# rpng/open_vins

Hardware: AMD Instinct MI355X
Metric: MSCKF features/sec per EKF update (30-clone state) (higher is better)
Workload: dtype f64; 1 GPU; BASELINE.json configs[2]: 2-camera radtan rig, 30-clone window, 2000 MSCKF features/update, N=248, D=208, online cam extrinsic+intrinsic calib + IMU intrinsics in the state, FEJ; features_total=2000, features_this_rank=2000, clones=30, cameras=2, state_dim=248, measurements_total=100362, parallelism=single GPU

## Files before the change

open_vins_amd/csrc/api_context.inc:

```
using namespace ovg;

static thread_local std::string g_err = "";
static int set_err(int code, const std::string &msg) {
  g_err = msg;
  return code;
}

#define HIPCHK(expr)                                                                                         \
  do {                                                                                                       \
    hipError_t _e = (expr);                                                                                  \
    if (_e != hipSuccess) {                                                                                  \
      return set_err(OVGPU_ERR_HIP, std::string(#expr) + " -> " + hipGetErrorString(_e) + " (" __FILE__ ":" + \
                                        std::to_string(__LINE__) + ")");                                     \
    }                                                                                                        \
  } while (0)

namespace {

struct AllocCount {
  std::atomic<int64_t> n{0}, bytes{0};
  void add(size_t b) { n.fetch_add(1, std::memory_order_relaxed), bytes.fetch_add((int64_t)b, std::memory_order_relaxed); }
  void sub(size_t b) { n.fetch_sub(1, std::memory_order_relaxed), bytes.fetch_sub((int64_t)b, std::memory_order_relaxed); }
};
struct DeviceAlloc {
// ... 354 lines not shown
  int chol_spin_limit = 1 << 22;
  int chol_timeouts = 0;
  int mode_a_factor = 0;
  bool factor_from_gram = false;
  bool last_factor_from_gram = false;
  int last_gram_kernel = 0, last_factor_kernel = 0, last_unwhiten_kernel = 0;
  bool chol_timed_out = false;
  bool prior_pending = false;
  bool prior_overlap = true;
  const double *last_uinv = nullptr;
  const double *prior_uinv = nullptr;
  int layout_fpw = 8;
  bool unwhiten_blocked = true;
  bool pchol_blocked = true;
  bool speculative_prior = true;
  DevBuf<int32_t> gram_dropped;
  DevView<int32_t> rows_used;
  DevBuf<double> sys_rows_ws;
  int row_stride = 48;

  std::vector<EventPair> ev_compress, ev_update, ev_system;
  size_t ev_used = 0;
  bool timed_this_update = false;
  bool timing = true;
  int timing_period = 1;
  uint64_t timing_seq = 0;
};

static Batch batch_of(const ovgpu_ctx *c) {
  if (c->view) return *c->view;
// ... 164 lines not shown
```

open_vins_amd/csrc/api_debug.inc:

```
int ovgpu_debug_option(ovgpu_ctx *c, const char *name, int64_t value, int64_t *old_value) {
  if (!c || !name) return set_err(OVGPU_ERR_INVALID, "null argument");
  const std::string n(name);
  if (n == "chol_follow_spin_limit") {
    if (old_value) *old_value = c->chol_spin_limit;
    if (value >= 0) c->chol_spin_limit = (int)std::min<int64_t>(value, 1 << 30);
  } else if (n == "slam_chunked_fail_chunk") {
    if (old_value) *old_value = c->chunk_fail_inject;
    c->chunk_fail_inject = value >= 0 ? (int)std::min<int64_t>(value, 1 << 20) : -1;
  } else if (n == "slam_chunked_fallbacks") {
    if (old_value) *old_value = c->chunk_fallbacks;
    if (value >= 0) c->chunk_fallbacks = value;
  } else if (n == "delayed_init_fused") {
    if (old_value) *old_value = c->init_fused;
    if (value >= 0) c->init_fused = (int)std::min<int64_t>(value, 2);
  } else if (n == "delayed_init_fused_steps") {
    if (old_value) *old_value = c->init_fused_steps;
    if (value >= 0) c->init_fused_steps = value;
  } else if (n == "delayed_init_rows_steps") {
    if (old_value) *old_value = c->init_rows_steps;
    if (value >= 0) c->init_rows_steps = value;
  } else if (n == "delayed_init_chain_steps") {
    if (old_value) *old_value = c->init_chain_steps;
    if (value >= 0) c->init_chain_steps = value;
  } else if (n == "gram_interleaved") {
    if (old_value) *old_value = c->gram_il ? 1 : 0;
    if (value >= 0) c->gram_il = value != 0;
  } else if (n == "layout_fpw") {
    if (old_value) *old_value = c->layout_fpw;
    if (value >= 1 && value <= 8) c->layout_fpw = (int)value;
  } else if (n == "unwhiten_blocked") {
    if (old_value) *old_value = c->unwhiten_blocked ? 1 : 0;
    if (value >= 0) c->unwhiten_blocked = value != 0;
  } else if (n == "pchol_blocked") {
    if (old_value) *old_value = c->pchol_blocked ? 1 : 0;
    if (value >= 0) c->pchol_blocked = value != 0;
  } else if (n == "speculative_prior") {
    if (old_value) *old_value = c->speculative_prior ? 1 : 0;
    if (value >= 0) c->speculative_prior = value != 0;
  } else if (n == "raw_stack") {
    if (old_value) *old_value = c->raw_enable ? 1 : 0;
    if (value >= 0) c->raw_enable = value != 0, c->raw_one_region = value == 2;
  } else if (n == "anchored_fast") {
    if (old_value) *old_value = c->anchored_fast ? 1 : 0;
    if (value >= 0) c->anchored_fast = value != 0;
  } else if (n == "slam_fused") {
    if (old_value) *old_value = c->slam_fused;
    if (value >= 0) c->slam_fused = (int)std::min<int64_t>(value, 3);
  } else if (n == "slam_fused_batches") {
    if (old_value) *old_value = c->slam_fused_batches;
    if (value >= 0) c->slam_fused_batches = value;
  } else if (n == "gram_blocks_only") {
    if (old_value) *old_value = c->gram_blocks_only ? 1 : 0;
    if (value >= 0) c->gram_blocks_only = value != 0;
// ... 279 lines not shown
```

open_vins_amd/csrc/api_pipeline.inc:

```
static int enqueue_triangulate(ovgpu_ctx *c, const double *seed_pA = nullptr, const int32_t *seed_anchor = nullptr) {
  const Batch b = batch_of(c);
  if (b.F == 0) return OVGPU_OK;
  TriParams p;
  p.seed_pA = seed_pA, p.seed_anchor = seed_anchor, p.anchor_pre = c->anchor_pre.p;
  p.F = b.F, p.C = c->C, p.K = c->K;
  p.meas_offsets = b.meas_offsets, p.meas_cc = b.meas_cc, p.uvn = b.uvn, p.tab_cc = c->tab_cc.p;
  p.p_FinA = b.pA, p.p_FinG = b.pG, p.anchor_meas = c->anchor.p, p.status = b.status;
  p.opt = c->dopt;
  const size_t lds = (size_t)c->K * c->C * 12 * sizeof(double);
  if (lds > (size_t)c->lds_limit) {
    return set_err(OVGPU_ERR_CAPACITY, "k_triangulate: the pose table of K = " + std::to_string(c->K) + " cameras x C = " + std::to_string(c->C) + " clones (96 bytes a pair, " +
                                           std::to_string(lds) + " bytes) exceeds the LDS limit of " + std::to_string(c->lds_limit) + " bytes");
  }
  int wpb = c->tri_waves;
  if (wpb == 0) {
    wpb = 4;
    const int room = c->num_cu - 6;
    for (int w = 4; w <= 8 && room > 0; w *= 2) {
      const int blocks = (b.F + w - 1) / w;
      if (blocks <= room) {
        if (4 * blocks >= 3 * room) wpb = w;
        break;
      }
    }
  }
  hipLaunchKernelGGL(with_max_lds<k_triangulate>(c), dim3((b.F + wpb - 1) / wpb), dim3(64 * wpb), lds, c->stream, p);
  HIPCHK(hipGetLastError());
  return OVGPU_OK;
}

struct FeatLaunch {
  FeatKernel kernel = FK_GENERAL;
  FeatKernel code = FK_GENERAL;
  bool f32 = false;
  bool ch = false;
  bool alt = false;
  int cb = 0;
  size_t lds = 0;
// ... 100 lines not shown

static int enqueue_system(ovgpu_ctx *c, int f_one = -1, int init_rep = 0, bool whiten = false) {
  const Batch b = batch_of(c);
  if (b.F == 0) return OVGPU_OK;
  SysParams p;
  fill_sys_params(c, b, p);
  c->stack_is_f32 = false;
  p.Lw = (whiten && f_one < 0) ? c->Lw.p : nullptr;
  c->last_stack_raw = false;
  if (f_one < 0) c->last_feat_kernel = FK_GENERAL;
  if (f_one < 0) HIPCHK(ctrl_zero(c, CTRL_ROWS, c->rows_used.p, 2 * sizeof(int32_t), c->stream));
  if (f_one >= 0) sys_params_init_mode(c, p, f_one, init_rep);
  const FeatLaunch s = select_feat_kernel(c, p, b.F, f_one);
  if (s.err != OVGPU_OK) return set_err(s.err, s.msg);
  if (s.cb) {
    p.row_stride = 48;
    HIPCHK(ctrl_zero(c, CTRL_COUNTER, c->feat_counter.p, sizeof(int32_t), c->stream));
    p.work_counter = c->feat_counter.p;
    feat::FeatStore st{c->fs_rows.p, c->fs_minfo.p, c->fs_V.p, c->fs_z.p, c->fs_meas_feat.p, c->fs_w.p, c->fs_pos.p};
    if (s.f32) {
      c->stack_ldf = ((c->LD + 31) / 32) * 32;
      HIPCHK(c->Hbig32.reserve((size_t)(std::max<int64_t>(b.rows_total, 1) + 32) * c->stack_ldf));
      HIPCHK(hipMemsetAsync(c->Hbig32.p + (size_t)b.rows_total * c->stack_ldf, 0, sizeof(float) * 32 * c->stack_ldf, c->stream));
      p.Hbig32 = c->Hbig32.p, p.LDF = c->stack_ldf;
      c->stack_is_f32 = true;
    }
    if (p.opt.feat_rep >= OVGPU_REP_ANCHORED_3D) hipLaunchKernelGGL(feat::k_feat_rows_anchored, dim3((b.M + 255) / 256), dim3(256), 0, c->stream, p, st, b.M);
    else hipLaunchKernelGGL(feat::k_feat_rows_sorted, dim3((b.M + 255) / 256), dim3(256), 0, c->stream, p, st, b.M);
    if (c->raw_enable && c->raw_tables_ok && !c->raw_veto && s.kernel != FK_FEATY_BIG && !s.f32 && s.cb == feat::FY_CB) {
      p.raw.on = 1, p.raw.ncls = c->raw_ncls, p.raw.H = c->Hraw.p, p.raw.dst = c->raw_dst.p, p.raw.j0 = c->raw_j0;
// ... 442 lines not shown
      sp = c->stream2;
      c->prior_on_side = true;
    }
    const int64_t elems = (int64_t)D * LA;
    const bool at_source = c->fuse_chol_inputs && chol_pipe_usable(c, D);
    if (!at_source) hipLaunchKernelGGL(k_tf_gather, dim3((unsigned)((elems + 255) / 256)), dim3(256), 0, sp, t);
    p.diag0 = c->gram_rho.p, p.pivot_tol = c->prior_pivot_tol;
    CholSource from;
    if (at_source) from.src = chol::CH_SRC_PRIOR, from.t = &t;
    c->last_uinv = nullptr;
    if ((rc = enqueue_chol_carry(c, p, sp, c->Lw.p, from)) != OVGPU_OK) return rc;
    c->prior_uinv = c->last_uinv;
    p.diag0 = nullptr;
    if (c->prior_on_side) HIPCHK(hipEventRecord(c->ev_join, sp));
    c->prior_pending = true;
  }
  if (part & 2) {
    if (c->prior_on_side) HIPCHK(hipStreamWaitEvent(s, c->ev_join, 0));
    c->prior_pending = false, c->prior_on_side = false;
    p.pred = c->flags.p + 3;
    CholSource from;
    if (t.whitened && c->fuse_chol_inputs && chol_pipe_usable(c, D)) {
      from.src = chol::CH_SRC_WHITENED, from.t = &t;
      p.pred = nullptr, p.pred_not = c->flags.p;
    } else if (t.whitened) {
      hipLaunchKernelGGL(k_tf_abh, dim3((D + 3) / 4), dim3(256), 0, s, t, (const int32_t *)c->flags.p, c->flags.p + 3);
    } else {
      hipLaunchKernelGGL(k_tf_go, dim3(1), dim3(1), 0, s, (const int32_t *)c->flags.p, c->flags.p + 3);
      hipLaunchKernelGGL(k_tf_w, dim3((tm * tm + 3) / 4), dim3(256), 0, s, t);
      hipLaunchKernelGGL(k_tf_t, dim3((tm * tm + 3) / 4), dim3(256), 0, s, t);
// ... 536 lines not shown
```

open_vins_amd/csrc/api_standalone.inc:

```
int ovgpu_measurement_compress(ovgpu_ctx *c, int rows, int cols, const double *H, const double *res, double *H_out, double *res_out, int32_t *rows_out) {
  if (!c) return set_err(OVGPU_ERR_INVALID, "null ctx");
  if (rows <= cols) {
    if (H_out && H && H_out != H) std::memcpy(H_out, H, sizeof(double) * (size_t)rows * cols);
    if (res_out && res && res_out != res) std::memcpy(res_out, res, sizeof(double) * rows);
    if (rows_out) *rows_out = rows;
    return OVGPU_OK;
  }
  DenseJob job(c);
  int rc = dense_compress(c, rows, cols, H, res);
  if (rc != OVGPU_OK) return rc;
  const int LD = cols + 1;
  std::vector<double> tri((size_t)cols * LD);
  HIPCHK(hipMemcpyAsync(tri.data(), c->Rws.p, sizeof(double) * tri.size(), hipMemcpyDeviceToHost, c->stream));
  HIPCHK(upload_sync(c, c->stream));
  for (int i = 0; i < cols; i++) {
    if (H_out) std::memcpy(H_out + (size_t)i * cols, &tri[(size_t)i * LD], sizeof(double) * cols);
    if (res_out) res_out[i] = tri[(size_t)i * LD + cols];
  }
  if (rows_out) *rows_out = cols;
  return check_tree_error(c);
}

int ovgpu_ekf_update(ovgpu_ctx *c, int rows, int cols, const int32_t *col_cov_id, const double *H, const double *res, double sigma2, double *dx,
                     double *P_out) {
// ... 56 lines not shown
  if (!c || !n_doubles) return set_err(OVGPU_ERR_INVALID, "null argument");
  if (!c->have_state || c->poses_only) return set_err(OVGPU_ERR_NO_STATE, "ovgpu_set_state was never called");
  const int NT = (c->LD + 15) / 16;
  if (NT > gram::GR_NT_BLK) return set_err(OVGPU_ERR_CAPACITY, "the Gram route holds at most 383 Jacobian columns");
  *n_doubles = (int64_t)256 * NT * NT + 1;
  return OVGPU_OK;
}

int ovgpu_msckf_local_gram(ovgpu_ctx *c, int32_t *feat_status, double *chi2, double *chi2_thresh, double *p_FinG, void *gram_dev,
                           ovgpu_update_stats *stats) {
  if (!c || !gram_dev) return set_err(OVGPU_ERR_INVALID, "null argument");
  if (stats) std::memset(stats, 0, sizeof(*stats));
  if (!c->have_state || c->poses_only) return set_err(OVGPU_ERR_NO_STATE, "ovgpu_set_state was never called");
  HIPCHK(hipSetDevice(c->device));
  int rc = OVGPU_OK;
  c->prior_pending = false;
  rc = enqueue_pipeline(c, STAGE_LOCAL, false, true, true);
  if (rc != OVGPU_OK) return rc;
  const size_t n = (size_t)256 * ((c->LD + 15) / 16) * ((c->LD + 15) / 16);
  double *dst = static_cast<double *>(gram_dev);
  if (batch_of(c).F > 0) {
    HIPCHK(hipMemcpyAsync(dst, c->gram_G.p, sizeof(double) * n, hipMemcpyDeviceToDevice, c->stream));
    hipLaunchKernelGGL(k_gram_count, dim3(1), dim3(1), 0, c->stream, dst + n, c->rows_used.p);
    HIPCHK(hipGetLastError());
  } else {
    HIPCHK(hipMemsetAsync(dst, 0, sizeof(double) * (n + 1), c->stream));
    c->gram_is_whitened = c->whiten;
  }
  if (feat_status || chi2 || chi2_thresh || p_FinG || stats) {
    rc = read_feature_outputs(c, feat_status, chi2, chi2_thresh, p_FinG, stats);
    if (rc != OVGPU_OK) return rc;
// ... 128 lines not shown
```

open_vins_amd/csrc/api_state.inc:

```

const char *ovgpu_last_error(void) { return g_err.c_str(); }

void ovgpu_default_options(ovgpu_options *o) {
  if (!o) return;
  std::memset(o, 0, sizeof(*o));
  o->chi2_multipler = 5.0, o->sigma_pix = 1.0;
  o->triangulate_1d = 0, o->refine_features = 1, o->max_runs = 5;
  o->init_lamda = 1e-3, o->max_lamda = 1e10, o->min_dx = 1e-6, o->min_dcost = 1e-6, o->lam_mult = 10;
  o->min_dist = 0.10, o->max_dist = 60, o->max_baseline = 40, o->max_cond_number = 10000;
  o->do_fej = 1, o->do_calib_camera_pose = 1, o->do_calib_camera_intrinsics = 1;
  o->feat_rep_msckf = OVGPU_REP_GLOBAL_3D;
}

double ovgpu_chi2_quantile_95(int dof) { return chi2_quantile_95(dof); }
int ovgpu_abi_version(void) { return OVGPU_ABI_VERSION; }

static int init_context(ovgpu_ctx *c, const ovgpu_options *opts, int device) {
  c->device = device;
  c->opts = *opts;
  hipDeviceProp_t prop;
  HIPCHK(hipGetDeviceProperties(&prop, device));
  c->num_cu = prop.multiProcessorCount > 0 ? prop.multiProcessorCount : 256;
  c->lds_limit = (int)std::min<size_t>(prop.sharedMemPerBlock, 160 * 1024);
  HIPCHK(hipStreamCreateWithFlags(&c->stream.h, hipStreamNonBlocking));
// ... 379 lines not shown
  std::vector<double> tab((size_t)12 * K * C);
  for (int i = 0; i < K * C; i++) {
    std::memcpy(&tab[(size_t)12 * i], R_GtoC + (size_t)9 * i, 9 * sizeof(double));
    std::memcpy(&tab[(size_t)12 * i + 9], p_CinG + (size_t)3 * i, 3 * sizeof(double));
  }
  HIPCHK(c->tab_cc.reserve(tab.size()));
  HIPCHK(upload(c->tab_cc.p, tab.data(), sizeof(double) * tab.size(), c->stream));
  HIPCHK(upload_sync(c, c->stream));
  c->C = C, c->K = K, c->N = 0, c->D = 0, c->LD = 1, c->L = 0;
  c->have_state = true, c->poses_only = true, c->have_feats = false, c->tri_readable = false;
  return OVGPU_OK;
}

static bool featy_block_rows(const ovgpu_ctx *c) { return c->plan.msckf == FK_FEATY_BIG || c->featy_big; }
static int featy_block_cols(const ovgpu_ctx *c) { return featy_block_rows(c) ? 32 : feat::FY_CB; }
static int enqueue_batch_layout(ovgpu_ctx *c, bool anchors, int cb) {
  const Batch b = batch_of(c);
  const int F = b.F;
  const bool fast = c->plan.msckf != FK_GENERAL && b.M > 0;
  if (F > 0 && (anchors || fast)) {
    const int m_max = feat::batch_layout_m_pad(std::max(b.m_max, 1));
    const size_t lds_one = feat::batch_layout_lds_ints(m_max) * sizeof(int32_t);
    int fpw_want = 1;
    while (fpw_want < std::min(c->layout_fpw, (int)feat::BL_FPW) && (F + fpw_want - 1) / fpw_want > 250) fpw_want *= 2;
    const int fpw = fast ? std::max(1, std::min<int>(fpw_want, (int)((48 * 1024) / lds_one))) : 1;
    const size_t lds = fast ? (size_t)fpw * lds_one : 0;
    const bool raw_tabs = fast && c->raw_tables_ok;
    RawStack rw;
    for (int k = 0; k <= RAW_NEG; k++) rw.base[k] = c->raw_base[k], rw.ld[k] = c->raw_ld[k], rw.rcol[k] = c->raw_rcol[k];
    hipLaunchKernelGGL(feat::k_batch_layout, dim3((F + fpw - 1) / fpw), dim3(fast ? feat::BL_NTH * fpw : 64), lds, c->stream, F, m_max, c->D, (const int32_t *)b.meas_offsets, (const uint16_t *)b.meas_cc,
                       (const int32_t *)c->clone_col.p, (const int32_t *)c->calib_col.p, (const int32_t *)c->intr_col.p, anchors ? c->anchor_pre.p : (int32_t *)nullptr,
                       fast ? c->fs_meas_feat.p : (int32_t *)nullptr, fast ? c->fs_pos.p : (int32_t *)nullptr, fast ? c->fs_inst.p : (int32_t *)nullptr, c->plan.nt, cb, c->C, c->K,
                       (const uint8_t *)c->cls_of_clone.p, (const int32_t *)c->raw_featbase.p, raw_tabs ? c->raw_dst.p : (int32_t *)nullptr,
                       raw_tabs ? c->raw_runs.p : (int32_t *)nullptr, rw);
    HIPCHK(hipGetLastError());
  }
  c->inst_cb = fast ? cb : 0, c->inst_D = c->D;
  return OVGPU_OK;
}
static int enqueue_instance_lists(ovgpu_ctx *c, int cb) { return enqueue_batch_layout(c, false, cb); }
static int enqueue_batch_tables(ovgpu_ctx *c, bool anchors) { return enqueue_batch_layout(c, anchors, c->plan.msckf != FK_GENERAL ? featy_block_cols(c) : feat::FY_CB); }

static int feature_rows(bool slam_rows, int m, int proj) { return slam_rows ? std::max(2 * m - proj, 0) : (m >= 2 ? 2 * m - 3 : 0); }
static void row_offsets_of(const ovgpu_ctx *c, const Batch &b, bool slam_rows, int64_t *out) {
  const int udof = lm_uniform_dof(c);
  out[0] = 0;
  for (int f = 0; f < b.F; f++) {
    int proj = udof == 1 ? 2 : 0;
    if (udof == 0 && (int)b.h_feat_lm.size() == b.F) proj = 3 - lm_dof(c->h_lm_rep[b.h_feat_lm[f]]);
    out[f + 1] = out[f] + feature_rows(slam_rows, b.h_offsets[f + 1] - b.h_offsets[f], proj);
  }
}
static void track_order(const int32_t *offsets, int F, int m_max, int32_t *order) {
  std::vector<int32_t> start(m_max + 2, 0);
  for (int f = 0; f < F; f++) start[m_max - (offsets[f + 1] - offsets[f]) + 1]++;
  for (int b = 0; b <= m_max; b++) start[b + 1] += start[b];
// ... 150 lines not shown
      r.chunk_begin = (int)((nchunks * j) / w), r.chunk_end = (int)((nchunks * (j + 1)) / w);
      r.part_tile = tiles, r.region = (c->raw_rs.n - 1) | (k == RAW_NEG ? 16 : 0);
      tiles += r.ntc * (r.ntc + 1) / 2;
      tab.push_back(r);
    }
  }
  c->gram_wg_n = (int)tab.size(), c->gram_wg_tiles = tiles;
  HIPCHK(c->gram_wg.reserve(tab.size()));
  HIPCHK(c->up.put(c->gram_wg.p, tab.data(), sizeof(gram::GramRegionWG) * tab.size()));
  c->raw_tables_ok = true;
  return OVGPU_OK;
}

static int begin_feature_batch(ovgpu_ctx *c, int F, int M, const int32_t *offsets) {
  c->have_feats = false, c->tri_readable = false;
  c->raw_tables_ok = false;
  int m_max = 0;
  for (int f = 0; f < F; f++) {
    const int m = offsets[f + 1] - offsets[f];
    if (m < 0) return set_err(OVGPU_ERR_INVALID, "meas_offsets not monotone");
    m_max = std::max(m_max, m);
  }
  c->F = F, c->M = M, c->m_max = m_max;
  c->have_feat_sigma = c->have_feat_mult = false;
  c->h_feat_lm.clear(), c->h_feat_rep.clear();
  c->h_offsets.assign(offsets, offsets + (F > 0 ? F + 1 : 0));
  if (F == 0) c->h_offsets.assign(1, 0);

  const int need = std::max(500, 2 * m_max + 1);
  if ((int)c->h_chi2_table.size() < need) {
// ... 87 lines not shown
```

open_vins_amd/csrc/k_featy.h:

```cpp
#pragma once
#include <type_traits>

#include "k_feat.h"

namespace ovg {
namespace feat {

#ifdef OVG_FEAT_ABLATE
#define FY_SKIP(p) ((p).skip)
#else
#define FY_SKIP(p) 0
#endif
#ifndef FY_SYRK_UNROLL
#define FY_SYRK_UNROLL 2
#endif
constexpr int FY_CB = 64;
constexpr int FY_LS = 66;

struct FeatYLds {
  size_t yb, vl, wpart, misc, raw, total;
};
__host__ __device__ inline FeatYLds featy_lds_layout(int nt_max, int nta_max, int nw, int cb) {
  FeatYLds L;
  size_t o = 0;
// ... 132 lines not shown
        p.raw.H[off + (int64_t)(r & 1) * ld + rcol] = res[r];
      }
      if (lane < 4) {
        const double cr = lane < 3 && lane < n ? res[lane] - (V[3 * lane] * z0 + V[3 * lane + 1] * z1 + V[3 * lane + 2] * z2) : 0.0;
        p.raw.H[p.raw.base[RAW_NEG] + ((int64_t)4 * f + lane) * p.raw.ld[RAW_NEG] + p.raw.rcol[RAW_NEG]] = cr;
      }
    }
    if (lane == 0) tq[(size_t)8 * f + 6] = sumsq / p.opt.sigma_pix_sq;
  }
}

__host__ __device__ inline int batch_layout_m_pad(int m_max) { return (m_max + 15) & ~15; }
__host__ __device__ inline size_t batch_layout_lds_ints(int m_pad) { return (size_t)4 * m_pad + (size_t)((2 * m_pad + 15) >> 4) * 48; }
constexpr int BL_NTH = 128, BL_TR = BL_NTH / 24;
constexpr int BL_FPW = 8;
__global__ void __launch_bounds__(BL_NTH * BL_FPW) k_batch_layout(int F, int m_max, int D, const int32_t *__restrict__ meas_offsets, const uint16_t *__restrict__ meas_cc,
                                                      const int32_t *__restrict__ clone_col, const int32_t *__restrict__ calib_col, const int32_t *__restrict__ intr_col,
                                                      int32_t *__restrict__ anchor_pre, int32_t *__restrict__ meas_feat, int32_t *__restrict__ pos, int32_t *__restrict__ inst,
                                                      int nt_max, int cb, int C, int K, const uint8_t *__restrict__ cls_of_clone, const int32_t *__restrict__ featbase,
                                                      int32_t *__restrict__ raw_dst, int32_t *__restrict__ raw_runs, RawStack rw) {
  extern __shared__ __attribute__((aligned(16))) unsigned char smem_all[];
  const int gth = min((int)blockDim.x, BL_NTH), grp = threadIdx.x / gth;
  const int tid = threadIdx.x - grp * gth, lane = tid & 63, wv = tid >> 6;
  const int f = blockIdx.x * ((int)blockDim.x / gth) + grp;
  const bool active = f < F;
  unsigned char *smem = smem_all + (size_t)grp * batch_layout_lds_ints(m_max) * sizeof(int32_t);
  __shared__ int tab_clone[1024], tab_calib[64], tab_intr[64];
  __shared__ uint8_t tab_cls[1024];
  __shared__ int grp_nt[BL_FPW];
  __shared__ __attribute__((aligned(16))) int cls_cnt[BL_FPW][RAW_MAXCLS];
  if (pos) {
    if (raw_runs && tid < RAW_MAXCLS) cls_cnt[grp][tid] = 0;
    for (int i = threadIdx.x; i < C; i += blockDim.x) tab_clone[i] = clone_col[i];
    if (raw_dst)
      for (int i = threadIdx.x; i < C; i += blockDim.x) tab_cls[i] = cls_of_clone[i];
    if (threadIdx.x < K) tab_calib[threadIdx.x] = calib_col[threadIdx.x], tab_intr[threadIdx.x] = intr_col[threadIdx.x];
  }
  const int m0 = active ? meas_offsets[f] : 0, m = active ? meas_offsets[f + 1] - m0 : 0;
  if (pos && tid == 0) grp_nt[grp] = (2 * m + 15) >> 4;
  if (anchor_pre && active && wv == (gth >> 6) - 1) {
    long long best = -1;
    int best_end = -1, carry_start = 0;
    for (int base = 0; base < m; base += 64) {
      const int i = base + lane;
      const bool valid = i < m;
      const int cam = valid ? (int)(meas_cc[m0 + i] >> 10) : -1;
      const int prev = (valid && i > 0) ? (int)(meas_cc[m0 + i - 1] >> 10) : -2;
      const int next = (valid && i + 1 < m) ? (int)(meas_cc[m0 + i + 1] >> 10) : -3;
      const unsigned long long starts = __ballot(valid && cam != prev);
      if (valid && cam != next) {
        const unsigned long long below = starts & (lane == 63 ? ~0ull : ((2ull << lane) - 1ull));
        const int start = below ? base + 63 - __clzll((long long)below) : carry_start;
        const long long key = ((long long)(i - start + 1) << 32) | (long long)(0x7fffffff - start);
        if (key > best) best = key, best_end = i;
      }
      if (starts) carry_start = base + 63 - __clzll((long long)starts);
    }
#pragma unroll
    for (int off = 32; off >= 1; off >>= 1) {
      const long long ob = __shfl_xor(best, off);
      const int oe = __shfl_xor(best_end, off);
      if (ob > best) best = ob, best_end = oe;
    }
    if (lane == 0) anchor_pre[f] = best_end >= 0 ? m0 + best_end : -1;
  }
  if (!pos) return;
  typedef int i32x4 __attribute__((ext_vector_type(4)));
  int *keys = reinterpret_cast<int *>(smem);
  int *cols3 = keys + m_max;
  int *cand = cols3 + 3 * m_max;
  const int NT = (2 * m + 15) >> 4;
  int *kept = cand + 24 * ((2 * m_max + 15) >> 4);
  __syncthreads();
  for (int i = tid; i < ((m + 15) & ~15); i += BL_NTH) {
    int key = 0x7fffffff;
    if (i < m) {
      const int code = meas_cc[m0 + i], cam = code >> 10;
      key = (tab_clone[code & 1023] << 8) | cam;
      meas_feat[m0 + i] = f;
      if (raw_runs) atomicAdd(&cls_cnt[grp][tab_cls[code & 1023]], 1);
      if (inst) cand[i] = tab_calib[cam], kept[i] = tab_intr[cam];
    }
    keys[i] = key;
  }
  __syncthreads();
  for (int i = tid; i < m; i += BL_NTH) {
    const int mykey = keys[i];
    int rank = 0;
    const i32x4 *k4 = reinterpret_cast<const i32x4 *>(keys);
    for (int j = 0; j < m; j += 16) {
      const i32x4 a = k4[(j >> 2)], b = k4[(j >> 2) + 1], c = k4[(j >> 2) + 2], d = k4[(j >> 2) + 3];
#define OVG_RK(v, o) rank += (v.x < mykey) || (v.x == mykey && j + o < i), rank += (v.y < mykey) || (v.y == mykey && j + o + 1 < i), \
                     rank += (v.z < mykey) || (v.z == mykey && j + o + 2 < i), rank += (v.w < mykey) || (v.w == mykey && j + o + 3 < i)
      OVG_RK(a, 0), OVG_RK(b, 4), OVG_RK(c, 8), OVG_RK(d, 12);
#undef OVG_RK
    }
    pos[m0 + i] = m0 + rank;
    if (raw_dst) {
      const int k = tab_cls[meas_cc[m0 + i] & 1023];
      raw_dst[m0 + rank] = (k << RAW_CLS_SHIFT) | (featbase[f * RAW_MAXCLS + k] + 2 * rank);
    }
    if (inst) {
      const int c1 = cand[i], c2 = kept[i];
      cols3[3 * rank] = mykey >> 8, cols3[3 * rank + 1] = c1, cols3[3 * rank + 2] = c2;
    }
  }
  if (raw_runs && active && tid >= BL_NTH - FY_RUNREC) {
    const int k = BL_NTH - 1 - tid;
    const i32x4 ca = *reinterpret_cast<const i32x4 *>(&cls_cnt[grp][0]), cb4 = *reinterpret_cast<const i32x4 *>(&cls_cnt[grp][4]);
    const int cn[RAW_MAXCLS] = {ca.x, ca.y, ca.z, ca.w, cb4.x, cb4.y, cb4.z, cb4.w};
    int lo = 0, mine = 0, above = 0, nr = 0;
#pragma unroll
    for (int j = 0; j < RAW_MAXCLS; j++) lo += j < k ? cn[j] : 0, mine = j == k ? cn[j] : mine, above += j > k && cn[j] > 0, nr += cn[j] > 0;
    i32x4 *rt = reinterpret_cast<i32x4 *>(raw_runs) + (size_t)f * FY_RUNREC;
    if (k == RAW_MAXCLS) rt[RAW_MAXCLS] = i32x4{nr, 0, 0, 0};
    else if (mine > 0) {
      int64_t base = rw.base[0];
      int ld = rw.ld[0], rcol = rw.rcol[0];
#pragma unroll
      for (int q = 1; q < RAW_MAXCLS; q++)
        if (k == q) base = rw.base[q], ld = rw.ld[q], rcol = rw.rcol[q];
      const int64_t off = base + (int64_t)(featbase[f * RAW_MAXCLS + k] + 2 * lo) * ld;
      rt[above] = i32x4{(2 * lo) | ((2 * (lo + mine)) << 16), ld | (rcol << 16), (int)(uint32_t)(uint64_t)off, (int)(uint32_t)((uint64_t)off >> 32)};
    }
  }
  if (!inst) return;
  __syncthreads();
  const int nblk = (D + cb - 1) / cb;
  int nt_wg = 0;
  for (int q = 0; q < (int)blockDim.x / gth; q++) nt_wg = max(nt_wg, grp_nt[q]);
  for (int t0 = 0; t0 < nt_wg; t0 += BL_TR) {
    const int g = tid / 24, jk = tid - 24 * g, tr = t0 + g;
    const bool live = g < BL_TR && tr < NT;
    const int i = 8 * tr + jk / 3, kind = jk - 3 * (jk / 3);
    int v = -1;
    if (live && i < m) v = cols3[3 * i + kind];
    if (live) cand[24 * tr + jk] = v;
    __syncthreads();
    bool keep = v >= 0;
    if (live) {
      const i32x4 *c4 = reinterpret_cast<const i32x4 *>(cand + 24 * tr);
      int u[24];
#pragma unroll
      for (int q = 0; q < 6; q++) {
        const i32x4 w = c4[q];
        u[4 * q] = w.x, u[4 * q + 1] = w.y, u[4 * q + 2] = w.z, u[4 * q + 3] = w.w;
      }
#pragma unroll
      for (int e = 0; e < 24; e++) keep = keep && (e >= jk || u[e] != v);
    }
    const int width = kind == 2 ? 8 : 6, code = v | (width << 16) | (kind << 24);
    if (live) kept[24 * tr + jk] = keep ? code : -1;
    __syncthreads();
    if (live) {
      const i32x4 *k4 = reinterpret_cast<const i32x4 *>(kept + 24 * tr);
      int u[24];
#pragma unroll
      for (int q = 0; q < 6; q++) {
        const i32x4 w = k4[q];
        u[4 * q] = w.x, u[4 * q + 1] = w.y, u[4 * q + 2] = w.z, u[4 * q + 3] = w.w;
      }
      int *gl = inst + ((size_t)f * nt_max + tr) * FY_ISTR;
      int below = 0, cnt = 0, lim = -1;
#pragma unroll
      for (int e = 0; e < 24; e++) {
        const bool on = u[e] >= 0;
        cnt += on;
        below += on && (u[e] & 0xffff) < v;
// ... 9 lines not shown
          if (kb < nblk) {
            const int c_lo = cb * kb;
            int e0 = 0, e1 = 0;
#pragma unroll
            for (int e = 0; e < 24; e++) {
              const int end = (u[e] & 0xffff) + ((u[e] >> 16) & 0xff) - 1;
              e0 += u[e] >= 0 && end < c_lo, e1 += u[e] >= 0 && end < c_lo + cb / 2;
            }
            packed |= (e0 | (e1 << 5)) << (10 * q);
          }
        }
        gl[1 + jk] = packed;
      }
    }
  }
}
#endif

__device__ __forceinline__ void lds_barrier() { asm volatile("s_waitcnt lgkmcnt(0)\n\ts_barrier" ::: "memory"); }

template <int MODE = 0>
__device__ __forceinline__ double gate_corner_chi2(const d4 &t, int q, int coff, bool two = false) {
  double v = t[0];
#pragma unroll
  for (int u = 1; u < 4; u++) v = q == u ? t[u] : v;
  if (MODE == 1 || (MODE == 2 && !two)) return -bcast_lane(v, coff);
  const double c00 = bcast_lane(v, coff), c01 = bcast_lane(v, coff + 1), c02 = bcast_lane(v, coff + 2), c03 = bcast_lane(v, coff + 3);
  const double c11 = bcast_lane(v, 16 + coff + 1), c12 = bcast_lane(v, 16 + coff + 2), c13 = bcast_lane(v, 16 + coff + 3);
  const double c22 = bcast_lane(v, 32 + coff + 2), c23 = bcast_lane(v, 32 + coff + 3), c33 = bcast_lane(v, 48 + coff + 3);
  const M3 Gm{-c11, -c12, -c13, -c12, -c22, -c23, -c13, -c23, MODE == 2 ? 1.0 : -c33};
// ... 498 lines not shown
```

open_vins_amd/csrc/k_triangulate.h:

```cpp
#pragma once
#include "device_math.h"
#include "ovgpu_types.h"

namespace ovg {

__device__ __forceinline__ void build_tables_item(int t, int C, int K, const double *clone_qp, const double *clone_fej, const double *calib_qp,
                                                  double *tab_clone, double *tab_cam, double *tab_cc) {
  if (t < C) {
    const double *q = clone_qp + 7 * t;
    const double *qf = clone_fej + 7 * t;
    double *o = tab_clone + 24 * t;
    store_m3(o, quat_2_Rot(q[0], q[1], q[2], q[3]));
    o[9] = q[4], o[10] = q[5], o[11] = q[6];
    store_m3(o + 12, quat_2_Rot(qf[0], qf[1], qf[2], qf[3]));
    o[21] = qf[4], o[22] = qf[5], o[23] = qf[6];
  }
  if (t < K) {
    const double *q = calib_qp + 7 * t;
    double *o = tab_cam + 12 * t;
    store_m3(o, quat_2_Rot(q[0], q[1], q[2], q[3]));
    o[9] = q[4], o[10] = q[5], o[11] = q[6];
  }
  if (t < K * C) {
    const int k = t / C, c = t % C;
// ... 36 lines not shown
    const int code = meas_cc[i];
    const RelPose rp = rel_pose(lds_cc, (code >> 10) * C + (code & 1023), R_GtoA, p_AinG);
    const V3 pA = -1.0 * mul(rp.R_AtoCi, rp.p_CiinA);
    const M3 &R = rp.R_AtoCi;
    const double hi1 = R.a00 * alpha + R.a01 * beta + R.a02 + rho * pA.x;
    const double hi2 = R.a10 * alpha + R.a11 * beta + R.a12 + rho * pA.y;
    const double hi3 = R.a20 * alpha + R.a21 * beta + R.a22 + rho * pA.z;
    const float2 z = uvn[i];
    const float r0 = sub_f32(z.x, (float)(hi1 / hi3)), r1 = sub_f32(z.y, (float)(hi2 / hi3));
    const float n = sqrtf_rn(add_f32(mul_f32(r0, r0), mul_f32(r1, r1)));
    err += (double)n * (double)n;
  }
  return wave_sum(err);
}

__global__ void __launch_bounds__(1024) k_triangulate(TriParams p) {
  extern __shared__ __attribute__((aligned(16))) double lds_cc[];
  for (int i = threadIdx.x; i < p.K * p.C * 12; i += blockDim.x) lds_cc[i] = p.tab_cc[i];
  __syncthreads();

  const int lane = threadIdx.x & 63;
  const int f = blockIdx.x * (blockDim.x >> 6) + (threadIdx.x >> 6);
  if (f >= p.F) return;
  const int m0 = p.meas_offsets[f], m1 = p.meas_offsets[f + 1];
  const int m = m1 - m0;
  const float2 *uvn = reinterpret_cast<const float2 *>(p.uvn);

  auto finish = [&](int status, int anchor, const V3 &pA, const V3 &pG) {
    if (lane == 0) {
      p.status[f] = status;
      p.anchor_meas[f] = anchor;
      p.p_FinA[3 * f + 0] = pA.x, p.p_FinA[3 * f + 1] = pA.y, p.p_FinA[3 * f + 2] = pA.z;
      p.p_FinG[3 * f + 0] = pG.x, p.p_FinG[3 * f + 1] = pG.y, p.p_FinG[3 * f + 2] = pG.z;
    }
  };
  const double qnan = __longlong_as_double(0x7ff8000000000000LL);
  const V3 vnan{qnan, qnan, qnan};
  if (m < 2) {
    finish(OVGPU_FEAT_TOO_FEW_MEAS, -1, vnan, vnan);
    return;
  }

  const bool seeded = p.seed_pA != nullptr;
  const int anchor = __builtin_amdgcn_readfirstlane(seeded ? p.seed_anchor[f] : p.anchor_pre[f]);
  if (seeded && (anchor < m0 || anchor >= m1)) {
    finish(OVGPU_FEAT_TRI_FAILED, -1, vnan, vnan);
    return;
  }
  const int acode = p.meas_cc[anchor];
  const int acc = (acode >> 10) * p.C + (acode & 1023);
  const M3 R_GtoA = load_m3(lds_cc + 12 * acc);
  const V3 p_AinG = load_v3(lds_cc + 12 * acc + 9);

  V3 p_f;
  if (seeded) {
    p_f = load_v3(p.seed_pA + 3 * f);
  } else if (!p.opt.triangulate_1d) {
    double A00 = 0, A01 = 0, A02 = 0, A11 = 0, A12 = 0, A22 = 0, b0 = 0, b1 = 0, b2 = 0;
    for (int i = m0 + lane; i < m1; i += 64) {
// ... 121 lines not shown
      const int code = p.meas_cc[i];
      const RelPose rp = rel_pose(lds_cc, (code >> 10) * p.C + (code & 1023), R_GtoA, p_AinG);
      const double d1 = dot(q1, rp.p_CiinA), d2 = dot(q2, rp.p_CiinA);
      base_line_max = fmax(base_line_max, sqrt(d1 * d1 + d2 * d2));
    }
    base_line_max = wave_max(base_line_max);
    if (p_FinA.z < p.opt.min_dist || p_FinA.z > p.opt.max_dist || (pn / base_line_max) > p.opt.max_baseline || isnan(pn)) {
      finish(OVGPU_FEAT_GN_FAILED, anchor, vnan, vnan);
      return;
    }
  }
  const V3 p_FinG = mulT(R_GtoA, p_FinA) + p_AinG;
  finish(OVGPU_FEAT_USED, anchor, p_FinA, p_FinG);
}

}
```

Before: 2.950 million features/s.

## Fuse batch-layout table construction into triangulation kernel via deferred tables

Defers the batch layout/table kernel launch and, when possible, runs it inside a combined triangulation kernel where half the waves triangulate and the other half build layout tables using wave-level sync. Triangulation computes the anchor inline via a shared rule helper instead of reading precomputed anchors, so it no longer depends on the layout kernel. This aims to remove one kernel launch and a serial dependency per update, at the cost of more LDS per block and heavier per-block work. The change also drops a reset of prior_pending in the standalone path and adds counters.

```diff
diff --git a/open_vins_amd/csrc/anchor_rule.h b/open_vins_amd/csrc/anchor_rule.h
--- /dev/null
+++ b/open_vins_amd/csrc/anchor_rule.h
@@ -0,0 +1,34 @@
+#pragma once
+#include <hip/hip_runtime.h>
+#include <cstdint>
+
+namespace ovg {
+
+__device__ __forceinline__ int anchor_by_rule(const uint16_t *__restrict__ meas_cc, int m0, int m, int lane) {
+  long long best = -1;
+  int best_end = -1, carry_start = 0;
+  for (int base = 0; base < m; base += 64) {
+    const int i = base + lane;
+    const bool valid = i < m;
+    const int cam = valid ? (int)(meas_cc[m0 + i] >> 10) : -1;
+    const int prev = (valid && i > 0) ? (int)(meas_cc[m0 + i - 1] >> 10) : -2;
+    const int next = (valid && i + 1 < m) ? (int)(meas_cc[m0 + i + 1] >> 10) : -3;
+    const unsigned long long starts = __ballot(valid && cam != prev);
+    if (valid && cam != next) {
+      const unsigned long long below = starts & (lane == 63 ? ~0ull : ((2ull << lane) - 1ull));
+      const int start = below ? base + 63 - __clzll((long long)below) : carry_start;
+      const long long key = ((long long)(i - start + 1) << 32) | (long long)(0x7fffffff - start);
+      if (key > best) best = key, best_end = i;
+    }
+    if (starts) carry_start = base + 63 - __clzll((long long)starts);
+  }
+#pragma unroll
+  for (int off = 32; off >= 1; off >>= 1) {
+    const long long ob = __shfl_xor(best, off);
+    const int oe = __shfl_xor(best_end, off);
+    if (ob > best) best = ob, best_end = oe;
+  }
+  return best_end >= 0 ? m0 + best_end : -1;
+}
+
+}
diff --git a/open_vins_amd/csrc/api_context.inc b/open_vins_amd/csrc/api_context.inc
--- a/open_vins_amd/csrc/api_context.inc
+++ b/open_vins_amd/csrc/api_context.inc
@@ -392,6 +392,10 @@
   bool unwhiten_blocked = true;
   bool pchol_blocked = true;
   bool speculative_prior = true;
+  bool tables_with_tri = true;
+  bool tables_pending = false, tables_pending_anchors = false;
+  int64_t layout_launches = 0;
+  int64_t prior_factorisations = 0;
   DevBuf<int32_t> gram_dropped;
   DevView<int32_t> rows_used;
   DevBuf<double> sys_rows_ws;
diff --git a/open_vins_amd/csrc/api_debug.inc b/open_vins_amd/csrc/api_debug.inc
--- a/open_vins_amd/csrc/api_debug.inc
+++ b/open_vins_amd/csrc/api_debug.inc
@@ -37,6 +37,13 @@
   } else if (n == "speculative_prior") {
     if (old_value) *old_value = c->speculative_prior ? 1 : 0;
     if (value >= 0) c->speculative_prior = value != 0;
+  } else if (n == "tables_with_tri") {
+    if (old_value) *old_value = c->tables_with_tri ? 1 : 0;
+    if (value >= 0) c->tables_with_tri = value != 0;
+  } else if (n == "layout_launches") {
+    if (old_value) *old_value = c->layout_launches;
+  } else if (n == "prior_factorisations") {
+    if (old_value) *old_value = c->prior_factorisations;
   } else if (n == "raw_stack") {
     if (old_value) *old_value = c->raw_enable ? 1 : 0;
     if (value >= 0) c->raw_enable = value != 0, c->raw_one_region = value == 2;
diff --git a/open_vins_amd/csrc/api_pipeline.inc b/open_vins_amd/csrc/api_pipeline.inc
--- a/open_vins_amd/csrc/api_pipeline.inc
+++ b/open_vins_amd/csrc/api_pipeline.inc
@@ -22,6 +22,20 @@
         if (4 * blocks >= 3 * room) wpb = w;
         break;
       }
+    }
+  }
+  if (c->tables_pending) {
+    p.anchor_pre = nullptr;
+    const bool fast = c->plan.msckf != FK_GENERAL && b.M > 0;
+    const feat::BatchLayoutArgs a = batch_layout_args(c, b, c->tables_pending_anchors, batch_tables_cb(c), fast);
+    const size_t lds_cc = ((lds + 15) / 16) * 16, lds_all = lds_cc + (size_t)wpb * feat::batch_layout_lds_ints(a.m_max) * sizeof(int32_t);
+    if (fast && !c->view && !seed_pA && wpb <= feat::BL_FPW && lds_all + sizeof(feat::BatchLayoutTabs) <= (size_t)c->lds_limit) {
+      hipLaunchKernelGGL(with_max_lds<k_tri_layout>(c), dim3((b.F + wpb - 1) / wpb), dim3(128 * wpb), lds_all, c->stream, p, a);
+      HIPCHK(hipGetLastError());
+      c->tables_pending = c->tables_pending_anchors = false;
+      c->inst_cb = a.cb, c->inst_D = c->D;
+      c->layout_launches++;
+      return OVGPU_OK;
     }
   }
   hipLaunchKernelGGL(with_max_lds<k_triangulate>(c), dim3((b.F + wpb - 1) / wpb), dim3(64 * wpb), lds, c->stream, p);
@@ -152,6 +166,10 @@
   const FeatLaunch s = select_feat_kernel(c, p, b.F, f_one);
   if (s.err != OVGPU_OK) return set_err(s.err, s.msg);
   if (s.cb) {
+    {
+      const int rcf = flush_pending_tables(c);
+      if (rcf != OVGPU_OK) return rcf;
+    }
     p.row_stride = 48;
     HIPCHK(ctrl_zero(c, CTRL_COUNTER, c->feat_counter.p, sizeof(int32_t), c->stream));
     p.work_counter = c->feat_counter.p;
@@ -624,6 +642,7 @@
     p.diag0 = nullptr;
     if (c->prior_on_side) HIPCHK(hipEventRecord(c->ev_join, sp));
     c->prior_pending = true;
+    c->prior_factorisations++;
   }
   if (part & 2) {
     if (c->prior_on_side) HIPCHK(hipStreamWaitEvent(s, c->ev_join, 0));
diff --git a/open_vins_amd/csrc/api_standalone.inc b/open_vins_amd/csrc/api_standalone.inc
--- a/open_vins_amd/csrc/api_standalone.inc
+++ b/open_vins_amd/csrc/api_standalone.inc
@@ -94,7 +94,6 @@
   if (!c->have_state || c->poses_only) return set_err(OVGPU_ERR_NO_STATE, "ovgpu_set_state was never called");
   HIPCHK(hipSetDevice(c->device));
   int rc = OVGPU_OK;
-  c->prior_pending = false;
   rc = enqueue_pipeline(c, STAGE_LOCAL, false, true, true);
   if (rc != OVGPU_OK) return rc;
   const size_t n = (size_t)256 * ((c->LD + 15) / 16) * ((c->LD + 15) / 16);
diff --git a/open_vins_amd/csrc/api_state.inc b/open_vins_amd/csrc/api_state.inc
--- a/open_vins_amd/csrc/api_state.inc
+++ b/open_vins_amd/csrc/api_state.inc
@@ -417,32 +417,64 @@
 
 static bool featy_block_rows(const ovgpu_ctx *c) { return c->plan.msckf == FK_FEATY_BIG || c->featy_big; }
 static int featy_block_cols(const ovgpu_ctx *c) { return featy_block_rows(c) ? 32 : feat::FY_CB; }
+static feat::BatchLayoutArgs batch_layout_args(const ovgpu_ctx *c, const Batch &b, bool anchors, int cb, bool fast) {
+  const bool raw_tabs = fast && c->raw_tables_ok;
+  feat::BatchLayoutArgs a;
+  a.F = b.F, a.m_max = feat::batch_layout_m_pad(std::max(b.m_max, 1)), a.D = c->D;
+  a.meas_offsets = b.meas_offsets, a.meas_cc = b.meas_cc;
+  a.clone_col = c->clone_col.p, a.calib_col = c->calib_col.p, a.intr_col = c->intr_col.p;
+  a.anchor_pre = anchors ? c->anchor_pre.p : nullptr;
+  a.meas_feat = fast ? c->fs_meas_feat.p : nullptr, a.pos = fast ? c->fs_pos.p : nullptr, a.inst = fast ? c->fs_inst.p : nullptr;
+  a.nt_max = c->plan.nt, a.cb = cb, a.C = c->C, a.K = c->K;
+  a.cls_of_clone = c->cls_of_clone.p, a.featbase = c->raw_featbase.p;
+  a.raw_dst = raw_tabs ? c->raw_dst.p : nullptr, a.raw_runs = raw_tabs ? c->raw_runs.p : nullptr;
+  for (int k = 0; k <= RAW_NEG; k++) a.rw.base[k] = c->raw_base[k], a.rw.ld[k] = c->raw_ld[k], a.rw.rcol[k] = c->raw_rcol[k];
+  return a;
+}
 static int enqueue_batch_layout(ovgpu_ctx *c, bool anchors, int cb) {
   const Batch b = batch_of(c);
   const int F = b.F;
   const bool fast = c->plan.msckf != FK_GENERAL && b.M > 0;
   if (F > 0 && (anchors || fast)) {
-    const int m_max = feat::batch_layout_m_pad(std::max(b.m_max, 1));
-    const size_t lds_one = feat::batch_layout_lds_ints(m_max) * sizeof(int32_t);
+    const feat::BatchLayoutArgs a = batch_layout_args(c, b, anchors, cb, fast);
+    const size_t lds_one = feat::batch_layout_lds_ints(a.m_max) * sizeof(int32_t);
     int fpw_want = 1;
     while (fpw_want < std::min(c->layout_fpw, (int)feat::BL_FPW) && (F + fpw_want - 1) / fpw_want > 250) fpw_want *= 2;
     const int fpw = fast ? std::max(1, std::min<int>(fpw_want, (int)((48 * 1024) / lds_one))) : 1;
     const size_t lds = fast ? (size_t)fpw * lds_one : 0;
-    const bool raw_tabs = fast && c->raw_tables_ok;
-    RawStack rw;
-    for (int k = 0; k <= RAW_NEG; k++) rw.base[k] = c->raw_base[k], rw.ld[k] = c->raw_ld[k], rw.rcol[k] = c->raw_rcol[k];
-    hipLaunchKernelGGL(feat::k_batch_layout, dim3((F + fpw - 1) / fpw), dim3(fast ? feat::BL_NTH * fpw : 64), lds, c->stream, F, m_max, c->D, (const int32_t *)b.meas_offsets, (const uint16_t *)b.meas_cc,
-                       (const int32_t *)c->clone_col.p, (const int32_t *)c->calib_col.p, (const int32_t *)c->intr_col.p, anchors ? c->anchor_pre.p : (int32_t *)nullptr,
-                       fast ? c->fs_meas_feat.p : (int32_t *)nullptr, fast ? c->fs_pos.p : (int32_t *)nullptr, fast ? c->fs_inst.p : (int32_t *)nullptr, c->plan.nt, cb, c->C, c->K,
-                       (const uint8_t *)c->cls_of_clone.p, (const int32_t *)c->raw_featbase.p, raw_tabs ? c->raw_dst.p : (int32_t *)nullptr,
-                       raw_tabs ? c->raw_runs.p : (int32_t *)nullptr, rw);
+    hipLaunchKernelGGL(feat::k_batch_layout, dim3((F + fpw - 1) / fpw), dim3(fast ? feat::BL_NTH * fpw : 64), lds, c->stream, a);
     HIPCHK(hipGetLastError());
+    c->layout_launches++;
   }
   c->inst_cb = fast ? cb : 0, c->inst_D = c->D;
   return OVGPU_OK;
 }
-static int enqueue_instance_lists(ovgpu_ctx *c, int cb) { return enqueue_batch_layout(c, false, cb); }
-static int enqueue_batch_tables(ovgpu_ctx *c, bool anchors) { return enqueue_batch_layout(c, anchors, c->plan.msckf != FK_GENERAL ? featy_block_cols(c) : feat::FY_CB); }
+static int batch_tables_cb(const ovgpu_ctx *c) { return c->plan.msckf != FK_GENERAL ? featy_block_cols(c) : feat::FY_CB; }
+static int flush_pending_tables(ovgpu_ctx *c) {
+  if (!c->tables_pending) return OVGPU_OK;
+  const bool anchors = c->tables_pending_anchors;
+  c->tables_pending = c->tables_pending_anchors = false;
+  const Batch *view = c->view;
+  c->view = nullptr;
+  const int rc = enqueue_batch_layout(c, anchors, batch_tables_cb(c));
+  c->view = view;
+  return rc;
+}
+static int enqueue_instance_lists(ovgpu_ctx *c, int cb) {
+  const int rcf = flush_pending_tables(c);
+  return rcf != OVGPU_OK ? rcf : enqueue_batch_layout(c, false, cb);
+}
+static int enqueue_batch_tables(ovgpu_ctx *c, bool anchors) {
+  if (c->tables_with_tri && !c->view) {
+    c->tables_pending_anchors = anchors || (c->tables_pending && c->tables_pending_anchors);
+    c->tables_pending = true;
+    c->inst_cb = 0, c->inst_D = c->D;
+    return OVGPU_OK;
+  }
+  if (c->tables_pending) anchors = anchors || c->tables_pending_anchors;
+  c->tables_pending = c->tables_pending_anchors = false;
+  return enqueue_batch_layout(c, anchors, batch_tables_cb(c));
+}
 
 static int feature_rows(bool slam_rows, int m, int proj) { return slam_rows ? std::max(2 * m - proj, 0) : (m >= 2 ? 2 * m - 3 : 0); }
 static void row_offsets_of(const ovgpu_ctx *c, const Batch &b, bool slam_rows, int64_t *out) {
@@ -623,6 +655,7 @@
 
 static int begin_feature_batch(ovgpu_ctx *c, int F, int M, const int32_t *offsets) {
   c->have_feats = false, c->tri_readable = false;
+  c->tables_pending = c->tables_pending_anchors = false;
   c->raw_tables_ok = false;
   int m_max = 0;
   for (int f = 0; f < F; f++) {
diff --git a/open_vins_amd/csrc/k_featy.h b/open_vins_amd/csrc/k_featy.h
--- a/open_vins_amd/csrc/k_featy.h
+++ b/open_vins_amd/csrc/k_featy.h
@@ -2,6 +2,7 @@
 #include <type_traits>
 
 #include "k_feat.h"
+#include "anchor_rule.h"
 
 namespace ovg {
 namespace feat {
@@ -170,55 +171,63 @@
 __host__ __device__ inline size_t batch_layout_lds_ints(int m_pad) { return (size_t)4 * m_pad + (size_t)((2 * m_pad + 15) >> 4) * 48; }
 constexpr int BL_NTH = 128, BL_TR = BL_NTH / 24;
 constexpr int BL_FPW = 8;
-__global__ void __launch_bounds__(BL_NTH * BL_FPW) k_batch_layout(int F, int m_max, int D, const int32_t *__restrict__ meas_offsets, const uint16_t *__restrict__ meas_cc,
-                                                      const int32_t *__restrict__ clone_col, const int32_t *__restrict__ calib_col, const int32_t *__restrict__ intr_col,
-                                                      int32_t *__restrict__ anchor_pre, int32_t *__restrict__ meas_feat, int32_t *__restrict__ pos, int32_t *__restrict__ inst,
-                                                      int nt_max, int cb, int C, int K, const uint8_t *__restrict__ cls_of_clone, const int32_t *__restrict__ featbase,
-                                                      int32_t *__restrict__ raw_dst, int32_t *__restrict__ raw_runs, RawStack rw) {
-  extern __shared__ __attribute__((aligned(16))) unsigned char smem_all[];
-  const int gth = min((int)blockDim.x, BL_NTH), grp = threadIdx.x / gth;
-  const int tid = threadIdx.x - grp * gth, lane = tid & 63, wv = tid >> 6;
-  const int f = blockIdx.x * ((int)blockDim.x / gth) + grp;
+struct BatchLayoutArgs {
+  int F, m_max, D;
+  const int32_t *meas_offsets;
+  const uint16_t *meas_cc;
+  const int32_t *clone_col, *calib_col, *intr_col;
+  int32_t *anchor_pre, *meas_feat, *pos, *inst;
+  int nt_max, cb, C, K;
+  const uint8_t *cls_of_clone;
+  const int32_t *featbase;
+  int32_t *raw_dst, *raw_runs;
+  RawStack rw;
+};
+struct BatchLayoutTabs {
+  int clone[1024], calib[64], intr[64];
+  uint8_t cls[1024];
+  int grp_nt[BL_FPW];
+  __attribute__((aligned(16))) int cls_cnt[BL_FPW][RAW_MAXCLS];
+};
+__device__ __forceinline__ void batch_layout_tables(BatchLayoutTabs &tb, const BatchLayoutArgs &a, int tix, int nth) {
+  if (!a.pos) return;
+  for (int i = tix; i < a.C; i += nth) tb.clone[i] = a.clone_col[i];
+  if (a.raw_dst)
+    for (int i = tix; i < a.C; i += nth) tb.cls[i] = a.cls_of_clone[i];
+  if (tix < a.K) tb.calib[tix] = a.calib_col[tix], tb.intr[tix] = a.intr_col[tix];
+}
+template <bool WV> __device__ __forceinline__ void bl_sync() {
+  if constexpr (WV) {
+    __builtin_amdgcn_fence(__ATOMIC_RELEASE, "workgroup");
+    __builtin_amdgcn_wave_barrier();
+    __builtin_amdgcn_fence(__ATOMIC_ACQUIRE, "workgroup");
+  } else {
+    __syncthreads();
+  }
+}
+template <bool WV>
+__device__ __forceinline__ void batch_layout_body(const BatchLayoutArgs &a, BatchLayoutTabs &tb, unsigned char *smem_all, int f, int grp, int ngrp, int tid, bool anchor_wave) {
+  constexpr int GTH = WV ? 64 : BL_NTH, TR = GTH / 24;
+  const int F = a.F, m_max = a.m_max, D = a.D, nt_max = a.nt_max, cb = a.cb;
+  const int32_t *__restrict__ meas_offsets = a.meas_offsets;
+  const uint16_t *__restrict__ meas_cc = a.meas_cc;
+  int32_t *__restrict__ anchor_pre = a.anchor_pre, *__restrict__ meas_feat = a.meas_feat, *__restrict__ pos = a.pos, *__restrict__ inst = a.inst;
+  const int32_t *__restrict__ featbase = a.featbase;
+  int32_t *__restrict__ raw_dst = a.raw_dst, *__restrict__ raw_runs = a.raw_runs;
+  const RawStack &rw = a.rw;
+  int *tab_clone = tb.clone, *tab_calib = tb.calib, *tab_intr = tb.intr;
+  uint8_t *tab_cls = tb.cls;
+  int *grp_nt = tb.grp_nt;
+  int(*cls_cnt)[RAW_MAXCLS] = tb.cls_cnt;
+  const int lane = tid & 63;
   const bool active = f < F;
   unsigned char *smem = smem_all + (size_t)grp * batch_layout_lds_ints(m_max) * sizeof(int32_t);
-  __shared__ int tab_clone[1024], tab_calib[64], tab_intr[64];
-  __shared__ uint8_t tab_cls[1024];
-  __shared__ int grp_nt[BL_FPW];
-  __shared__ __attribute__((aligned(16))) int cls_cnt[BL_FPW][RAW_MAXCLS];
-  if (pos) {
-    if (raw_runs && tid < RAW_MAXCLS) cls_cnt[grp][tid] = 0;
-    for (int i = threadIdx.x; i < C; i += blockDim.x) tab_clone[i] = clone_col[i];
-    if (raw_dst)
-      for (int i = threadIdx.x; i < C; i += blockDim.x) tab_cls[i] = cls_of_clone[i];
-    if (threadIdx.x < K) tab_calib[threadIdx.x] = calib_col[threadIdx.x], tab_intr[threadIdx.x] = intr_col[threadIdx.x];
-  }
+  if (pos && raw_runs && tid < RAW_MAXCLS) cls_cnt[grp][tid] = 0;
   const int m0 = active ? meas_offsets[f] : 0, m = active ? meas_offsets[f + 1] - m0 : 0;
   if (pos && tid == 0) grp_nt[grp] = (2 * m + 15) >> 4;
-  if (anchor_pre && active && wv == (gth >> 6) - 1) {
-    long long best = -1;
-    int best_end = -1, carry_start = 0;
-    for (int base = 0; base < m; base += 64) {
-      const int i = base + lane;
-      const bool valid = i < m;
-      const int cam = valid ? (int)(meas_cc[m0 + i] >> 10) : -1;
-      const int prev = (valid && i > 0) ? (int)(meas_cc[m0 + i - 1] >> 10) : -2;
-      const int next = (valid && i + 1 < m) ? (int)(meas_cc[m0 + i + 1] >> 10) : -3;
-      const unsigned long long starts = __ballot(valid && cam != prev);
-      if (valid && cam != next) {
-        const unsigned long long below = starts & (lane == 63 ? ~0ull : ((2ull << lane) - 1ull));
-        const int start = below ? base + 63 - __clzll((long long)below) : carry_start;
-        const long long key = ((long long)(i - start + 1) << 32) | (long long)(0x7fffffff - start);
-        if (key > best) best = key, best_end = i;
-      }
-      if (starts) carry_start = base + 63 - __clzll((long long)starts);
-    }
-#pragma unroll
-    for (int off = 32; off >= 1; off >>= 1) {
-      const long long ob = __shfl_xor(best, off);
-      const int oe = __shfl_xor(best_end, off);
-      if (ob > best) best = ob, best_end = oe;
-    }
-    if (lane == 0) anchor_pre[f] = best_end >= 0 ? m0 + best_end : -1;
+  if (anchor_pre && active && anchor_wave) {
+    const int am = anchor_by_rule(meas_cc, m0, m, lane);
+    if (lane == 0) anchor_pre[f] = am;
   }
   if (!pos) return;
   typedef int i32x4 __attribute__((ext_vector_type(4)));
@@ -227,8 +236,8 @@
   int *cand = cols3 + 3 * m_max;
   const int NT = (2 * m + 15) >> 4;
   int *kept = cand + 24 * ((2 * m_max + 15) >> 4);
-  __syncthreads();
-  for (int i = tid; i < ((m + 15) & ~15); i += BL_NTH) {
+  bl_sync<WV>();
+  for (int i = tid; i < ((m + 15) & ~15); i += GTH) {
     int key = 0x7fffffff;
     if (i < m) {
       const int code = meas_cc[m0 + i], cam = code >> 10;
@@ -239,16 +248,16 @@
     }
     keys[i] = key;
   }
-  __syncthreads();
-  for (int i = tid; i < m; i += BL_NTH) {
+  bl_sync<WV>();
+  for (int i = tid; i < m; i += GTH) {
     const int mykey = keys[i];
     int rank = 0;
     const i32x4 *k4 = reinterpret_cast<const i32x4 *>(keys);
     for (int j = 0; j < m; j += 16) {
-      const i32x4 a = k4[(j >> 2)], b = k4[(j >> 2) + 1], c = k4[(j >> 2) + 2], d = k4[(j >> 2) + 3];
+      const i32x4 a4 = k4[(j >> 2)], b = k4[(j >> 2) + 1], c = k4[(j >> 2) + 2], d = k4[(j >> 2) + 3];
 #define OVG_RK(v, o) rank += (v.x < mykey) || (v.x == mykey && j + o < i), rank += (v.y < mykey) || (v.y == mykey && j + o + 1 < i), \
                      rank += (v.z < mykey) || (v.z == mykey && j + o + 2 < i), rank += (v.w < mykey) || (v.w == mykey && j + o + 3 < i)
-      OVG_RK(a, 0), OVG_RK(b, 4), OVG_RK(c, 8), OVG_RK(d, 12);
+      OVG_RK(a4, 0), OVG_RK(b, 4), OVG_RK(c, 8), OVG_RK(d, 12);
 #undef OVG_RK
     }
     pos[m0 + i] = m0 + rank;
@@ -261,8 +270,8 @@
       cols3[3 * rank] = mykey >> 8, cols3[3 * rank + 1] = c1, cols3[3 * rank + 2] = c2;
     }
   }
-  if (raw_runs && active && tid >= BL_NTH - FY_RUNREC) {
-    const int k = BL_NTH - 1 - tid;
+  if (raw_runs && active && tid >= GTH - FY_RUNREC) {
+    const int k = GTH - 1 - tid;
     const i32x4 ca = *reinterpret_cast<const i32x4 *>(&cls_cnt[grp][0]), cb4 = *reinterpret_cast<const i32x4 *>(&cls_cnt[grp][4]);
     const int cn[RAW_MAXCLS] = {ca.x, ca.y, ca.z, ca.w, cb4.x, cb4.y, cb4.z, cb4.w};
     int lo = 0, mine = 0, above = 0, nr = 0;
@@ -281,18 +290,19 @@
     }
   }
   if (!inst) return;
-  __syncthreads();
+  bl_sync<WV>();
   const int nblk = (D + cb - 1) / cb;
-  int nt_wg = 0;
-  for (int q = 0; q < (int)blockDim.x / gth; q++) nt_wg = max(nt_wg, grp_nt[q]);
-  for (int t0 = 0; t0 < nt_wg; t0 += BL_TR) {
+  int nt_wg = WV ? NT : 0;
+  if constexpr (!WV)
+    for (int q = 0; q < ngrp; q++) nt_wg = max(nt_wg, grp_nt[q]);
+  for (int t0 = 0; t0 < nt_wg; t0 += TR) {
     const int g = tid / 24, jk = tid - 24 * g, tr = t0 + g;
-    const bool live = g < BL_TR && tr < NT;
+    const bool live = g < TR && tr < NT;
     const int i = 8 * tr + jk / 3, kind = jk - 3 * (jk / 3);
     int v = -1;
     if (live && i < m) v = cols3[3 * i + kind];
     if (live) cand[24 * tr + jk] = v;
-    __syncthreads();
+    bl_sync<WV>();
     bool keep = v >= 0;
     if (live) {
       const i32x4 *c4 = reinterpret_cast<const i32x4 *>(cand + 24 * tr);
@@ -307,7 +317,7 @@
     }
     const int width = kind == 2 ? 8 : 6, code = v | (width << 16) | (kind << 24);
     if (live) kept[24 * tr + jk] = keep ? code : -1;
-    __syncthreads();
+    bl_sync<WV>();
     if (live) {
       const i32x4 *k4 = reinterpret_cast<const i32x4 *>(kept + 24 * tr);
       int u[24];
@@ -347,6 +357,14 @@
       }
     }
   }
+}
+__global__ void __launch_bounds__(BL_NTH * BL_FPW) k_batch_layout(BatchLayoutArgs a) {
+  extern __shared__ __attribute__((aligned(16))) unsigned char smem_all[];
+  __shared__ BatchLayoutTabs tabs;
+  const int gth = min((int)blockDim.x, BL_NTH), grp = threadIdx.x / gth, ngrp = (int)blockDim.x / gth;
+  const int tid = threadIdx.x - grp * gth;
+  batch_layout_tables(tabs, a, threadIdx.x, blockDim.x);
+  batch_layout_body<false>(a, tabs, smem_all, blockIdx.x * ngrp + grp, grp, ngrp, tid, (tid >> 6) == (gth >> 6) - 1);
 }
 #endif
 
diff --git a/open_vins_amd/csrc/k_triangulate.h b/open_vins_amd/csrc/k_triangulate.h
--- a/open_vins_amd/csrc/k_triangulate.h
+++ b/open_vins_amd/csrc/k_triangulate.h
@@ -1,6 +1,10 @@
 #pragma once
 #include "device_math.h"
 #include "ovgpu_types.h"
+#include "anchor_rule.h"
+#ifndef OVG_TU_FEATY
+#include "k_featy.h"
+#endif
 
 namespace ovg {
 
@@ -74,14 +78,7 @@
   return wave_sum(err);
 }
 
-__global__ void __launch_bounds__(1024) k_triangulate(TriParams p) {
-  extern __shared__ __attribute__((aligned(16))) double lds_cc[];
-  for (int i = threadIdx.x; i < p.K * p.C * 12; i += blockDim.x) lds_cc[i] = p.tab_cc[i];
-  __syncthreads();
-
-  const int lane = threadIdx.x & 63;
-  const int f = blockIdx.x * (blockDim.x >> 6) + (threadIdx.x >> 6);
-  if (f >= p.F) return;
+__device__ __forceinline__ void triangulate_feature(const TriParams &p, const double *lds_cc, int f, int lane) {
   const int m0 = p.meas_offsets[f], m1 = p.meas_offsets[f + 1];
   const int m = m1 - m0;
   const float2 *uvn = reinterpret_cast<const float2 *>(p.uvn);
@@ -102,7 +99,7 @@
   }
 
   const bool seeded = p.seed_pA != nullptr;
-  const int anchor = __builtin_amdgcn_readfirstlane(seeded ? p.seed_anchor[f] : p.anchor_pre[f]);
+  const int anchor = __builtin_amdgcn_readfirstlane(seeded ? p.seed_anchor[f] : (p.anchor_pre ? p.anchor_pre[f] : anchor_by_rule(p.meas_cc, m0, m, lane)));
   if (seeded && (anchor < m0 || anchor >= m1)) {
     finish(OVGPU_FEAT_TRI_FAILED, -1, vnan, vnan);
     return;
@@ -254,4 +251,35 @@
   finish(OVGPU_FEAT_USED, anchor, p_FinA, p_FinG);
 }
 
-}
+__global__ void __launch_bounds__(1024) k_triangulate(TriParams p) {
+  extern __shared__ __attribute__((aligned(16))) double lds_cc[];
+  for (int i = threadIdx.x; i < p.K * p.C * 12; i += blockDim.x) lds_cc[i] = p.tab_cc[i];
+  __syncthreads();
+
+  const int lane = threadIdx.x & 63;
+  const int f = blockIdx.x * (blockDim.x >> 6) + (threadIdx.x >> 6);
+  if (f >= p.F) return;
+  triangulate_feature(p, lds_cc, f, lane);
+}
+
+#ifndef OVG_TU_FEATY
+__global__ void __launch_bounds__(1024) k_tri_layout(TriParams p, feat::BatchLayoutArgs a) {
+  extern __shared__ __attribute__((aligned(16))) double lds_cc[];
+  __shared__ feat::BatchLayoutTabs tabs;
+  const int ncc = p.K * p.C * 12;
+  for (int i = threadIdx.x; i < ncc; i += blockDim.x) lds_cc[i] = p.tab_cc[i];
+  feat::batch_layout_tables(tabs, a, threadIdx.x, blockDim.x);
+  __syncthreads();
+
+  const int lane = threadIdx.x & 63, w = blockDim.x >> 7, wv = threadIdx.x >> 6;
+  const int f = blockIdx.x * w + (wv < w ? wv : wv - w);
+  if (wv < w) {
+    if (f < p.F) triangulate_feature(p, lds_cc, f, lane);
+    return;
+  }
+  unsigned char *smem = reinterpret_cast<unsigned char *>(lds_cc + ((ncc + 1) & ~1));
+  feat::batch_layout_body<true>(a, tabs, smem, f, wv - w, w, lane, true);
+}
+#endif
+
+}
```

Result: no change. 2.949 million features/s (-0.0%).
